# Wu0409/DuPL

Measured on AMD Instinct MI355X. Metric: training img/s at 448^2, VOC dual-student ViT-B/16, phase B step, higher is better.
Workload: dtype f32 storage / accumulation / results; Linear GEMMs (forward, dgrad, wgrad), attention (forward, backward) and the decoder convs as fp32-equivalent f16x3 split products on the f16 MFMA (operands as fp16 hi / lo planes, 3 products per block, fp32 accumulate; error vs fp64 <= the f32 MFMA kernels'); CA

## Files before the change

### dupl_amd/csrc/attn_split.hip

```cpp
#include "split_frag.h"
#include "../../include/dupl_hip.h"

#ifndef ATT_PRIO
#define ATT_PRIO 0
#endif
#ifndef ATT_ABL
#define ATT_ABL 0
#endif

namespace {

constexpr int HD = 64, KT = 64;
constexpr int PLANE = KT * 128;
constexpr int STAGE = 4 * PLANE;

struct AttnSegs {
    int n;
    int row0[DUPL_ATTN_SEGS_MAX], B[DUPL_ATTN_SEGS_MAX], N[DUPL_ATTN_SEGS_MAX], B_f32[DUPL_ATTN_SEGS_MAX], first[DUPL_ATTN_SEGS_MAX + 1];
    float* out[DUPL_ATTN_SEGS_MAX];
    float* lse[DUPL_ATTN_SEGS_MAX];
};

template <class In, class Out>
__device__ __forceinline__ void attn_seg_planes(const size_t r0, const int H, In& qkv_hi, In& qkv_lo, Out& out_hi, Out& out_lo) {
    qkv_hi += r0 * (size_t)(3 * H * HD);
    qkv_lo += r0 * (size_t)(3 * H * HD);
    if (out_hi) { out_hi += r0 * (size_t)(H * HD); out_lo += r0 * (size_t)(H * HD); }
}

__global__ __launch_bounds__(256, 2) void attn_fwd16_kernel(const __half* __restrict__ qkv_hi, const __half* __restrict__ qkv_lo,
                                                            __half* __restrict__ out_hi, __half* __restrict__ out_lo,
                                                            const AttnSegs segs, int H, float scale, int remap, float out_scale) {
    __shared__ __attribute__((aligned(1024))) char smem[2 * STAGE];
    const int tid = threadIdx.x, lane = tid & 63, l31 = lane & 31, hf = lane >> 5;
    const int wave = __builtin_amdgcn_readfirstlane(tid >> 6);
    int sg = 0;
#pragma unroll 1
    while (sg + 1 < segs.n && (int)blockIdx.x >= segs.first[sg + 1]) ++sg;
    sg = __builtin_amdgcn_readfirstlane(sg);
    const int N = segs.N[sg], B_f32 = segs.B_f32[sg];
    float* __restrict__ out = segs.out[sg];
    float* __restrict__ lse = segs.lse[sg];
    int bx, h, b;
    {
        const int gx = (N + 127) / 128;
        const int G = gx * H * segs.B[sg];
        const int L = (int)blockIdx.x - segs.first[sg];
        const int w = remap ? xcd_band(L, G) : L;
        bx = w % gx; h = (w / gx) % H; b = w / (gx * H);
    }
    attn_seg_planes((size_t)segs.row0[sg], H, qkv_hi, qkv_lo, out_hi, out_lo);
    const int q0 = bx * 128 + wave * 32;
    const int D = H * HD, ld = 3 * D;
    const int qrow = q0 + l31;
    const bool wave_active = q0 < N;

    h8 qh[4], ql[4];
    {
        const size_t off = ((size_t)b * N + min(qrow, N - 1)) * ld + h * HD + 8 * hf;
#pragma unroll
        for (int s = 0; s < 4; ++s) {
            qh[s] = load_bfrag(qkv_hi + off, s);
            ql[s] = load_bfrag(qkv_lo + off, s);
        }
    }

    const int prow = lane >> 3;
    const char* kbase[2];
    kbase[0] = reinterpret_cast<const char*>(qkv_hi + (size_t)b * N * ld + D + h * HD);
    kbase[1] = reinterpret_cast<const char*>(qkv_lo + (size_t)b * N * ld + D + h * HD);
    const char* vbase[2];
    vbase[0] = kbase[0] + D * 2;
    vbase[1] = kbase[1] + D * 2;
    int krow[2], kch[2], vrow[2];
    const int vch = km_piece_col_bytes(lane);
#pragma unroll
    for (int j = 0; j < 2; ++j) {
        const int r = 8 * (wave + 4 * j) + prow;
        krow[j] = r;
        kch[j] = rm_piece_col_bytes(lane, r);
        const int q = wave + 4 * j, srow = (lane >> 2) & 7;
        vrow[j] = (q >> 1) * 16 + (srow >> 2) * 8 + (q & 1) * 4 + (srow & 3);
    }
    const size_t tstride = (size_t)KT * ld * 2;
    unsigned koff[2], voff[2];
#pragma unroll
    for (int j = 0; j < 2; ++j) {
        koff[j] = (unsigned)krow[j] * (unsigned)(ld * 2) + kch[j];
        voff[j] = (unsigned)vrow[j] * (unsigned)(ld * 2) + vch;
    }
    auto dma16o = [](const char* ubase, const unsigned off, char* dst) __attribute__((always_inline)) { dma16(ubase + off, dst); };
    auto issue = [&](int t, int buf) __attribute__((always_inline)) {
        char* dst = smem + buf * STAGE + wave * 1024;
        const size_t o = t * tstride;
        if (t * KT + KT <= N) {
#pragma unroll
            for (int i = 0; i < 4; ++i) dma16o(kbase[i >> 1] + o, koff[i & 1], dst + i * 4096);
#pragma unroll
            for (int i = 0; i < 4; ++i) dma16o(vbase[i >> 1] + o, voff[i & 1], dst + (4 + i) * 4096);
        } else {
#pragma unroll
            for (int i = 0; i < 4; ++i)
                dma16o(kbase[i >> 1] + o, (unsigned)(min(t * KT + krow[i & 1], N - 1) - t * KT) * (unsigned)(ld * 2) + kch[i & 1], dst + i * 4096);
#pragma unroll
            for (int i = 0; i < 4; ++i)
                dma16o(vbase[i >> 1] + o, (unsigned)(min(t * KT + vrow[i & 1], N - 1) - t * KT) * (unsigned)(ld * 2) + vch, dst + (4 + i) * 4096);
        }
    };

    const int krow_a = pi_row(l31);
    const int k_off = krow_a * 128, k_sw = (krow_a >> 1) & 7;
    const int vg = lane >> 4, vq = lane & 15;
    const unsigned v_lds = (unsigned)(uintptr_t)((__attribute__((address_space(3))) char*)smem) + 2 * PLANE +
                           ((vg >> 1) * 4 + (vq >> 2)) * 64 + (16 * (vg & 1) + 4 * (vq & 3)) * 2;

    f32x16 oM[2], oX[2];
#pragma unroll
    for (int d = 0; d < 2; ++d)
#pragma unroll
        for (int e = 0; e < 16; ++e) { oM[d][e] = 0.f; oX[d][e] = 0.f; }
    float m_run = -INFINITY, l_run = 0.f;

    const int nkt = (N + KT - 1) / KT;
    long long tph[4] = {0, 0, 0, 0}, tlast = 0;
    constexpr bool ABL16 = ATT_ABL & 16;
    if (ABL16) tlast = clock64();
#define ATT_STAMP(i)                                  \
    if (ABL16) {                                      \
        const long long now_ = clock64();             \
        tph[i] += now_ - tlast;                       \
        tlast = now_;                                 \
    }
    issue(0, 0);
    for (int t = 0; t < nkt; ++t) {
        asm volatile("s_waitcnt vmcnt(0)" ::: "memory");
        __syncthreads();
        if (t + 1 < nkt) issue(t + 1, (t + 1) & 1);
        if (!wave_active) continue;
        const char* st = smem + (t & 1) * STAGE;
        ATT_STAMP(0)

        f32x16 sM[2], sX[2];
        const f32x16 zero16 = {0.f, 0.f, 0.f, 0.f, 0.f, 0.f, 0.f, 0.f, 0.f, 0.f, 0.f, 0.f, 0.f, 0.f, 0.f, 0.f};
        h8 kh[2][2], kl[2][2];
        auto k_read = [&](const int sstep, h8(&fh)[2], h8(&fl)[2]) __attribute__((always_inline)) {
            const int ch = ((2 * sstep + hf) ^ k_sw) * 16;
#pragma unroll
            for (int kt2 = 0; kt2 < 2; ++kt2) {
                fh[kt2] = *reinterpret_cast<const h8*>(st + kt2 * 4096 + k_off + ch);
                fl[kt2] = *reinterpret_cast<const h8*>(st + PLANE + kt2 * 4096 + k_off + ch);
            }
        };
        k_read(0, kh[0], kl[0]);
        __builtin_amdgcn_s_setprio(ATT_PRIO);
#pragma unroll
        for (int sstep = 0; sstep < 4; ++sstep) {
            const int cur = sstep & 1;
            if (sstep + 1 < 4) k_read(sstep + 1, kh[cur ^ 1], kl[cur ^ 1]);
            __builtin_amdgcn_sched_barrier(0);
            sM[0] = MFMA16(kh[cur][0], qh[sstep], sstep == 0 ? zero16 : sM[0]);
            sM[1] = MFMA16(kh[cur][1], qh[sstep], sstep == 0 ? zero16 : sM[1]);
            sX[0] = MFMA16(kh[cur][0], ql[sstep], sstep == 0 ? zero16 : sX[0]);
            sX[1] = MFMA16(kh[cur][1], ql[sstep], sstep == 0 ? zero16 : sX[1]);
            sX[0] = MFMA16(kl[cur][0], qh[sstep], sX[0]);
            sX[1] = MFMA16(kl[cur][1], qh[sstep], sX[1]);
            __builtin_amdgcn_sched_barrier(0);
        }
        __builtin_amdgcn_s_setprio(0);
        if (ATT_ABL & 16) { asm volatile("" ::"v"(sM[0]), "v"(sM[1]), "v"(sX[0]), "v"(sX[1])); }
        ATT_STAMP(1)
        h4 vf[2][8];
        const unsigned v_st = v_lds + (t & 1) * STAGE;
        auto v_read = [&](auto sgc, h4(&f)[8]) __attribute__((always_inline)) {
            constexpr int SG = decltype(sgc)::value;
            static_for<8>([&](auto ic) __attribute__((always_inline)) {
                constexpr int i = decltype(ic)::value, pl = i >> 2, dd = (i >> 1) & 1, jj = i & 1;
                f[i] = km_tr_read<pl * PLANE + ((SG * 2 + jj) * 2 + dd) * 512>(v_st);
            });
        };
        v_read(std::integral_constant<int, 0>{}, vf[0]);
        const float c1 = scale * 1.4426950408889634f, c2 = c1 * LO_INV;
        if (t == nkt - 1) {
            const int kbase_t = t * KT + 8 * hf;
#pragma unroll
            for (int kt2 = 0; kt2 < 2; ++kt2)
#pragma unroll
                for (int e = 0; e < 16; ++e)
                    if (kbase_t + 32 * kt2 + 16 * (e >> 3) + (e & 7) >= N) sM[kt2][e] = -INFINITY;
        }
        float mx = -INFINITY;
#pragma unroll
        for (int kt2 = 0; kt2 < 2; ++kt2)
#pragma unroll
            for (int e = 0; e < 16; ++e) mx = fmaxf(mx, sM[kt2][e]);
        {
            typedef unsigned u2v __attribute__((ext_vector_type(2)));
            const u2v sw = __builtin_amdgcn_permlane32_swap(__float_as_uint(mx), __float_as_uint(mx), false, false);
            mx = fmaxf(__uint_as_float(sw[0]), __uint_as_float(sw[1])) * c1;
        }
        const float m_cand = fmaxf(m_run, mx);
        const bool move = __builtin_amdgcn_ballot_w64(m_cand - m_run > 8.f) != 0;
        const float m_run2 = move ? m_cand : m_run;
        const float m_new = m_run2 == -INFINITY ? 0.f : m_run2;
        const float alpha = __builtin_amdgcn_exp2f(m_run - m_new);
        f32x2 psum2 = {0.f, 0.f};
        h8 ph[4], pl[4];
#pragma unroll
        for (int kt2 = 0; kt2 < 2; ++kt2)
#pragma unroll
            for (int e = 0; e < 16; e += 2) {
                const f32x2 m2 = {sM[kt2][e], sM[kt2][e + 1]}, x2 = {sX[kt2][e], sX[kt2][e + 1]};
                const f32x2 v2 = __builtin_elementwise_fma(x2, f32x2{c2, c2}, __builtin_elementwise_fma(m2, f32x2{c1, c1}, f32x2{-m_new, -m_new}));
                const f32x2 p2 = {__builtin_amdgcn_exp2f(v2[0]), __builtin_amdgcn_exp2f(v2[1])};
                psum2 += p2;
                split_pair(p2, ph[2 * kt2 + (e >> 3)], pl[2 * kt2 + (e >> 3)], e & 7);
            }
        const float psum = psum2[0] + psum2[1];
        l_run = l_run * alpha + psum;
        if (move) {
#pragma unroll
            for (int d = 0; d < 2; ++d)
#pragma unroll
                for (int e = 0; e < 16; ++e) { oM[d][e] *= alpha; oX[d][e] *= alpha; }
        }
        m_run = m_run2;
        if (ATT_ABL & 16) { asm volatile("" ::"v"(ph[0]), "v"(ph[3]), "v"(pl[0]), "v"(pl[3]), "v"(oM[0]), "v"(oX[1])); }
        ATT_STAMP(2)
        __builtin_amdgcn_s_setprio(ATT_PRIO);
        static_for<4>([&](auto sgc) __attribute__((always_inline)) {
            constexpr int sg = decltype(sgc)::value, cur = sg & 1;
            if constexpr (sg + 1 < 4) {
                v_read(std::integral_constant<int, sg + 1>{}, vf[cur ^ 1]);
                asm volatile("s_waitcnt lgkmcnt(8)" ::: "memory");
            } else {
                asm volatile("s_waitcnt lgkmcnt(0)" ::: "memory");
            }
            __builtin_amdgcn_sched_barrier(0);
            const h4(&f)[8] = vf[cur];
            const h8 vh0 = __builtin_shufflevector(f[0], f[1], 0, 1, 2, 3, 4, 5, 6, 7), vh1 = __builtin_shufflevector(f[2], f[3], 0, 1, 2, 3, 4, 5, 6, 7);
            const h8 vl0 = __builtin_shufflevector(f[4], f[5], 0, 1, 2, 3, 4, 5, 6, 7), vl1 = __builtin_shufflevector(f[6], f[7], 0, 1, 2, 3, 4, 5, 6, 7);
            oM[0] = MFMA16(vh0, ph[sg], oM[0]);
            oM[1] = MFMA16(vh1, ph[sg], oM[1]);
            oX[0] = MFMA16(vh0, pl[sg], oX[0]);
            oX[1] = MFMA16(vh1, pl[sg], oX[1]);
            oX[0] = MFMA16(vl0, ph[sg], oX[0]);
            oX[1] = MFMA16(vl1, ph[sg], oX[1]);
            __builtin_amdgcn_sched_barrier(0);
        });
        __builtin_amdgcn_s_setprio(0);
        if (ATT_ABL & 16) { asm volatile("" ::"v"(oM[0]), "v"(oM[1]), "v"(oX[0]), "v"(oX[1])); }
        ATT_STAMP(3)
    }
    if ((ATT_ABL & 16) && lse && tid == 0) {
        long long* q = reinterpret_cast<long long*>(lse + (((size_t)segs.B[sg] * H * N + 1) & ~(size_t)1)) +
                       (size_t)((int)blockIdx.x - segs.first[sg]) * 4;
        q[0] = tph[0]; q[1] = tph[1]; q[2] = tph[2]; q[3] = tph[3];
    }
    if (!wave_active) return;
    const float l_tot = l_run + __shfl_xor(l_run, 32, 64);
    const float inv = 1.f / l_tot;
    if (b >= B_f32) { out = nullptr; lse = nullptr; }
    if (qrow < N) {
        const size_t ro = ((size_t)b * N + qrow) * D + h * HD;
#pragma unroll
        for (int d = 0; d < 2; ++d)
#pragma unroll
            for (int g = 0; g < 4; ++g) {
                float v[4];
#pragma unroll
                for (int j = 0; j < 4; ++j) v[j] = (oM[d][4 * g + j] + oX[d][4 * g + j] * LO_INV) * inv;
                const int col = d * 32 + 8 * g + 4 * hf;
                if (out) *reinterpret_cast<float4*>(out + ro + col) = make_float4(v[0], v[1], v[2], v[3]);
                if (out_hi) {
                    __half hh[4], ll[4];
#pragma unroll
                    for (int j = 0; j < 4; ++j) {
                        if (out_scale > 0.f) split_f32_u(v[j] * out_scale, hh[j], ll[j]);
                        else split_f32(v[j], hh[j], ll[j]);
                    }
                    *reinterpret_cast<uint2*>(out_hi + ro + col) = *reinterpret_cast<const uint2*>(hh);
                    *reinterpret_cast<uint2*>(out_lo + ro + col) = *reinterpret_cast<const uint2*>(ll);
                }
            }
        if (lse && hf == 0) lse[((size_t)b * H + h) * N + qrow] = m_run * 0.6931471805599453f + logf(l_tot);
    }
}

template <int NP>
__global__ __launch_bounds__(256, 2) void attn_fwd16_m16_kernel(const __half* __restrict__ qkv_hi, const __half* __restrict__ qkv_lo,
                                                                __half* __restrict__ out_hi, __half* __restrict__ out_lo,
                                                                const AttnSegs segs, int H, float scale, int remap, float out_scale) {
    static_assert(NP == 1 || NP == 3, "one product or the three of f16x3");
    constexpr bool X = NP == 3;
    constexpr int PL = X ? 2 : 1;
    constexpr int STAGE = 2 * PL * PLANE;
    constexpr bool ABL16 = X && (ATT_ABL & 16);
    __shared__ __attribute__((aligned(1024))) char smem[2 * STAGE];
    const int tid = threadIdx.x, lane = tid & 63, c16 = lane & 15, g4 = lane >> 4;
    const int wave = __builtin_amdgcn_readfirstlane(tid >> 6);
    int sg = 0;
#pragma unroll 1
    while (sg + 1 < segs.n && (int)blockIdx.x >= segs.first[sg + 1]) ++sg;
    sg = __builtin_amdgcn_readfirstlane(sg);
    const int N = segs.N[sg], B_f32 = segs.B_f32[sg];
    float* __restrict__ out = segs.out[sg];
    float* __restrict__ lse = X ? segs.lse[sg] : nullptr;
    int bx, h, b;
    {
        const int gx = (N + 127) / 128;
        const int G = gx * H * segs.B[sg];
        const int L = (int)blockIdx.x - segs.first[sg];
        const int w = remap ? xcd_band(L, G) : L;
        bx = w % gx; h = (w / gx) % H; b = w / (gx * H);
    }
    attn_seg_planes((size_t)segs.row0[sg], H, qkv_hi, qkv_lo, out_hi, out_lo);
    const int q0 = bx * 128 + wave * 32;
    const int D = H * HD, ld = 3 * D;
    const bool wave_active = q0 < N;

    h8 qh[2][2], ql[2][2];
#pragma unroll
    for (int ct = 0; ct < 2; ++ct) {
        const size_t off = ((size_t)b * N + min(q0 + 16 * ct + c16, N - 1)) * ld + h * HD + 8 * g4;
#pragma unroll
        for (int ks = 0; ks < 2; ++ks) {
            qh[ct][ks] = load_bfrag(qkv_hi + off, 2 * ks);
            if constexpr (X) ql[ct][ks] = load_bfrag(qkv_lo + off, 2 * ks);
        }
    }

    const int prow = lane >> 3;
    const char* kbase[2];
    kbase[0] = reinterpret_cast<const char*>(qkv_hi + (size_t)b * N * ld + D + h * HD);
    kbase[1] = reinterpret_cast<const char*>(qkv_lo + (size_t)b * N * ld + D + h * HD);
    const char* vbase[2];
    vbase[0] = kbase[0] + D * 2;
    vbase[1] = kbase[1] + D * 2;
    int krow[2], kch[2], vrow[2];
    const int vch = km16_piece_col_bytes(wave, lane);
#pragma unroll
    for (int j = 0; j < 2; ++j) {
        krow[j] = 8 * (wave + 4 * j) + prow;
        kch[j] = rm16_piece_col_bytes(lane, krow[j]);
        vrow[j] = km16_piece_row(wave + 4 * j, lane);
    }
    const size_t tstride = (size_t)KT * ld * 2;
    unsigned koff[2], voff[2];
#pragma unroll
    for (int j = 0; j < 2; ++j) {
        koff[j] = (unsigned)krow[j] * (unsigned)(ld * 2) + kch[j];
        voff[j] = (unsigned)vrow[j] * (unsigned)(ld * 2) + vch;
    }
    auto dma16o = [](const char* ubase, const unsigned off, char* dst) __attribute__((always_inline)) { dma16(ubase + off, dst); };
    auto issue = [&](int t, int buf) __attribute__((always_inline)) {
        char* dst = smem + buf * STAGE + wave * 1024;
        const size_t o = t * tstride;
        if (t * KT + KT <= N) {
#pragma unroll
            for (int i = 0; i < 2 * PL; ++i) dma16o(kbase[i >> 1] + o, koff[i & 1], dst + i * 4096);
#pragma unroll
            for (int i = 0; i < 2 * PL; ++i) dma16o(vbase[i >> 1] + o, voff[i & 1], dst + (2 * PL + i) * 4096);
        } else {
#pragma unroll
            for (int i = 0; i < 2 * PL; ++i)
                dma16o(kbase[i >> 1] + o, (unsigned)(min(t * KT + krow[i & 1], N - 1) - t * KT) * (unsigned)(ld * 2) + kch[i & 1], dst + i * 4096);
#pragma unroll
            for (int i = 0; i < 2 * PL; ++i)
                dma16o(vbase[i >> 1] + o, (unsigned)(min(t * KT + vrow[i & 1], N - 1) - t * KT) * (unsigned)(ld * 2) + vch, dst + (2 * PL + i) * 4096);
        }
    };

    const int k_off = pi16_row(c16, 0) * 128 + ((g4 ^ rm16_swizzle(pi16_row(c16, 0))) * 16);
    const unsigned v_lds = (unsigned)(uintptr_t)((__attribute__((address_space(3))) char*)smem) + PL * PLANE + km16_read_lane_off(lane);

    f32x4 oM[4][2], oX[4][2];
#pragma unroll
    for (int d = 0; d < 4; ++d)
#pragma unroll
        for (int ct = 0; ct < 2; ++ct) { oM[d][ct] = f32x4{0.f, 0.f, 0.f, 0.f}; oX[d][ct] = f32x4{0.f, 0.f, 0.f, 0.f}; }
    float m_run[2] = {-INFINITY, -INFINITY}, l_run[2] = {0.f, 0.f};

    const int nkt = (N + KT - 1) / KT;
    long long tph[4] = {0, 0, 0, 0}, tlast = 0;
    if (ABL16) tlast = clock64();
    issue(0, 0);
    for (int t = 0; t < nkt; ++t) {
        asm volatile("s_waitcnt vmcnt(0)" ::: "memory");
        __syncthreads();
        if (t + 1 < nkt) issue(t + 1, (t + 1) & 1);
        if (!wave_active) continue;
        const char* st = smem + (t & 1) * STAGE;
        ATT_STAMP(0)

        f32x4 sM[2][2][2], sX[2][2][2];
        const f32x4 zero4 = {0.f, 0.f, 0.f, 0.f};
        h8 kh[2][2], kl[2][2];
        auto k_read = [&](const int step, h8(&fh)[2], h8(&fl)[2]) __attribute__((always_inline)) {
            const int a = (k_off ^ ((step & 1) * 64)) + (step >> 1) * 4096;
#pragma unroll
            for (int j = 0; j < 2; ++j) {
                fh[j] = *reinterpret_cast<const h8*>(st + a + j * 512);
                if constexpr (X) fl[j] = *reinterpret_cast<const h8*>(st + PLANE + a + j * 512);
            }
        };
        k_read(0, kh[0], kl[0]);
        if constexpr (X) __builtin_amdgcn_s_setprio(ATT_PRIO);
#pragma unroll
        for (int step = 0; step < 4; ++step) {
            const int cur = step & 1, G = step >> 1, ks = step & 1;
            if (step + 1 < 4) k_read(step + 1, kh[cur ^ 1], kl[cur ^ 1]);
            __builtin_amdgcn_sched_barrier(0);
#pragma unroll
            for (int j = 0; j < 2; ++j)
#pragma unroll
                for (int ct = 0; ct < 2; ++ct) sM[G][j][ct] = MFMA_16x16x32(kh[cur][j], qh[ct][ks], ks == 0 ? zero4 : sM[G][j][ct]);
            if constexpr (X) {
#pragma unroll
                for (int j = 0; j < 2; ++j)
#pragma unroll
                    for (int ct = 0; ct < 2; ++ct) sX[G][j][ct] = MFMA_16x16x32(kh[cur][j], ql[ct][ks], ks == 0 ? zero4 : sX[G][j][ct]);
#pragma unroll
                for (int j = 0; j < 2; ++j)
#pragma unroll
                    for (int ct = 0; ct < 2; ++ct) sX[G][j][ct] = MFMA_16x16x32(kl[cur][j], qh[ct][ks], sX[G][j][ct]);
            }
            __builtin_amdgcn_sched_barrier(0);
        }
        if constexpr (X) __builtin_amdgcn_s_setprio(0);
        if (ABL16) {
#pragma unroll
            for (int G = 0; G < 2; ++G)
#pragma unroll
                for (int j = 0; j < 2; ++j) asm volatile("" ::"v"(sM[G][j][0]), "v"(sM[G][j][1]), "v"(sX[G][j][0]), "v"(sX[G][j][1]));
        }
        ATT_STAMP(1)
        h4 vf[2][4 * PL];
        const unsigned v_st = v_lds + (t & 1) * STAGE;
        auto v_read = [&](auto hc, h4(&f)[4 * PL]) __attribute__((always_inline)) {
            constexpr int HS = decltype(hc)::value, S = HS >> 1, DH = HS & 1;
            static_for<4 * PL>([&](auto ic) __attribute__((always_inline)) {
                constexpr int i = decltype(ic)::value, pl = i >> 2, dd = (i >> 1) & 1, jj = i & 1;
                f[i] = km_tr_read<pl * PLANE + ((S * 2 + jj) * 4 + 2 * DH + dd) * 512>(v_st);
            });
        };
        v_read(std::integral_constant<int, 0>{}, vf[0]);
        const float c1 = scale * 1.4426950408889634f, c2 = c1 * LO_INV;
        if (t == nkt - 1) {
            const int kbase_t = t * KT + 8 * g4;
#pragma unroll
            for (int G = 0; G < 2; ++G)
#pragma unroll
                for (int j = 0; j < 2; ++j)
#pragma unroll
                    for (int i = 0; i < 4; ++i)
                        if (kbase_t + 32 * G + 4 * j + i >= N) { sM[G][j][0][i] = -INFINITY; sM[G][j][1][i] = -INFINITY; }
        }
        float mxp[2];
        bool want = false;
#pragma unroll
        for (int ct = 0; ct < 2; ++ct) {
            float mx = -INFINITY;
#pragma unroll
            for (int G = 0; G < 2; ++G)
#pragma unroll
                for (int j = 0; j < 2; ++j)
#pragma unroll
                    for (int i = 0; i < 4; ++i) mx = fmaxf(mx, sM[G][j][ct][i]);
            mxp[ct] = mx * c1;
            want = want || (fmaxf(m_run[ct], mxp[ct]) - m_run[ct] > 8.f);
        }
        const bool move = __builtin_amdgcn_ballot_w64(want) != 0;
        if (move) {
#pragma unroll
            for (int ct = 0; ct < 2; ++ct) {
                float mx = mxp[ct];
                mx = fmaxf(mx, __shfl_xor(mx, 16, 64));
                mx = fmaxf(mx, __shfl_xor(mx, 32, 64));
                const float m2 = fmaxf(m_run[ct], mx);
                const float alpha = __builtin_amdgcn_exp2f(m_run[ct] - (m2 == -INFINITY ? 0.f : m2));
                m_run[ct] = m2;
                l_run[ct] *= alpha;
#pragma unroll
                for (int d = 0; d < 4; ++d) {
                    oM[d][ct] *= alpha;
                    if constexpr (X) oX[d][ct] *= alpha;
                }
            }
        }
        h8 ph[2][2], pl[2][2];
#pragma unroll
        for (int ct = 0; ct < 2; ++ct) {
            const float m_new = m_run[ct] == -INFINITY ? 0.f : m_run[ct];
            f32x2 psum2 = {0.f, 0.f};
#pragma unroll
            for (int G = 0; G < 2; ++G)
#pragma unroll
                for (int j = 0; j < 2; ++j)
#pragma unroll
                    for (int i = 0; i < 4; i += 2) {
                        const f32x2 m2 = {sM[G][j][ct][i], sM[G][j][ct][i + 1]};
                        f32x2 v2;
                        if constexpr (X) {
                            const f32x2 x2 = {sX[G][j][ct][i], sX[G][j][ct][i + 1]};
                            v2 = __builtin_elementwise_fma(x2, f32x2{c2, c2}, __builtin_elementwise_fma(m2, f32x2{c1, c1}, f32x2{-m_new, -m_new}));
                        } else v2 = __builtin_elementwise_fma(m2, f32x2{c1, c1}, f32x2{-m_new, -m_new});
                        const f32x2 p2 = {__builtin_amdgcn_exp2f(v2[0]), __builtin_amdgcn_exp2f(v2[1])};
                        psum2 += p2;
                        if constexpr (X) split_pair(p2, ph[G][ct], pl[G][ct], 4 * j + i);
                        else {
                            const h2v hh = __builtin_convertvector(p2, h2v);
                            ph[G][ct][4 * j + i] = hh[0];
                            ph[G][ct][4 * j + i + 1] = hh[1];
                        }
                    }
            l_run[ct] += psum2[0] + psum2[1];
        }
        if (ABL16) {
            asm volatile("" ::"v"(ph[0][0]), "v"(ph[1][1]), "v"(pl[0][0]), "v"(pl[1][1]), "v"(oM[0][0]), "v"(oX[3][1]));
        }
        ATT_STAMP(2)
        if constexpr (X) __builtin_amdgcn_s_setprio(ATT_PRIO);
        static_for<4>([&](auto hc) __attribute__((always_inline)) {
            constexpr int hs = decltype(hc)::value, cur = hs & 1, S = hs >> 1, d0 = 2 * (hs & 1);
            if constexpr (hs + 1 < 4) {
                v_read(std::integral_constant<int, hs + 1>{}, vf[cur ^ 1]);
                if constexpr (X) asm volatile("s_waitcnt lgkmcnt(8)" ::: "memory");
                else asm volatile("s_waitcnt lgkmcnt(4)" ::: "memory");
            } else {
                asm volatile("s_waitcnt lgkmcnt(0)" ::: "memory");
            }
            __builtin_amdgcn_sched_barrier(0);
            const h4(&f)[4 * PL] = vf[cur];
            const h8 vh0 = __builtin_shufflevector(f[0], f[1], 0, 1, 2, 3, 4, 5, 6, 7), vh1 = __builtin_shufflevector(f[2], f[3], 0, 1, 2, 3, 4, 5, 6, 7);
            oM[d0][0] = MFMA_16x16x32(vh0, ph[S][0], oM[d0][0]);
            oM[d0][1] = MFMA_16x16x32(vh0, ph[S][1], oM[d0][1]);
            oM[d0 + 1][0] = MFMA_16x16x32(vh1, ph[S][0], oM[d0 + 1][0]);
            oM[d0 + 1][1] = MFMA_16x16x32(vh1, ph[S][1], oM[d0 + 1][1]);
            if constexpr (X) {
                const h8 vl0 = __builtin_shufflevector(f[4], f[5], 0, 1, 2, 3, 4, 5, 6, 7), vl1 = __builtin_shufflevector(f[6], f[7], 0, 1, 2, 3, 4, 5, 6, 7);
            oX[d0][0] = MFMA_16x16x32(vh0, pl[S][0], oX[d0][0]);
            oX[d0][1] = MFMA_16x16x32(vh0, pl[S][1], oX[d0][1]);
            oX[d0 + 1][0] = MFMA_16x16x32(vh1, pl[S][0], oX[d0 + 1][0]);
            oX[d0 + 1][1] = MFMA_16x16x32(vh1, pl[S][1], oX[d0 + 1][1]);
            oX[d0][0] = MFMA_16x16x32(vl0, ph[S][0], oX[d0][0]);
            oX[d0][1] = MFMA_16x16x32(vl0, ph[S][1], oX[d0][1]);
            oX[d0 + 1][0] = MFMA_16x16x32(vl1, ph[S][0], oX[d0 + 1][0]);
            oX[d0 + 1][1] = MFMA_16x16x32(vl1, ph[S][1], oX[d0 + 1][1]);
            }
            __builtin_amdgcn_sched_barrier(0);
        });
        if constexpr (X) __builtin_amdgcn_s_setprio(0);
        if (ABL16) {
#pragma unroll
            for (int d = 0; d < 4; ++d) asm volatile("" ::"v"(oM[d][0]), "v"(oM[d][1]), "v"(oX[d][0]), "v"(oX[d][1]));
        }
        ATT_STAMP(3)
    }
    if ((ABL16) && lse && tid == 0) {
        long long* q = reinterpret_cast<long long*>(lse + (((size_t)segs.B[sg] * H * N + 1) & ~(size_t)1)) +
                       (size_t)((int)blockIdx.x - segs.first[sg]) * 4;
        q[0] = tph[0]; q[1] = tph[1]; q[2] = tph[2]; q[3] = tph[3];
    }
    if (!wave_active) return;
    if (b >= B_f32) { out = nullptr; lse = nullptr; }
#pragma unroll
    for (int ct = 0; ct < 2; ++ct) {
        float l_tot = l_run[ct];
        l_tot += __shfl_xor(l_tot, 16, 64);
        l_tot += __shfl_xor(l_tot, 32, 64);
        const float inv = 1.f / l_tot;
        const int qrow = q0 + 16 * ct + c16;
        if (qrow < N) {
            const size_t ro = ((size_t)b * N + qrow) * D + h * HD;
#pragma unroll
            for (int d = 0; d < 4; ++d) {
                float v[4];
#pragma unroll
                for (int j = 0; j < 4; ++j) v[j] = (X ? oM[d][ct][j] + oX[d][ct][j] * LO_INV : oM[d][ct][j]) * inv;
                const int col = 16 * d + 4 * g4;
                if (out) *reinterpret_cast<float4*>(out + ro + col) = make_float4(v[0], v[1], v[2], v[3]);
                if (out_hi) {
                    __half hh[4], ll[4];
#pragma unroll
                    for (int j = 0; j < 4; ++j) {
                        if (out_scale > 0.f) split_f32_u(v[j] * out_scale, hh[j], ll[j]);
                        else split_f32(v[j], hh[j], ll[j]);
                    }
                    *reinterpret_cast<uint2*>(out_hi + ro + col) = *reinterpret_cast<const uint2*>(hh);
                    *reinterpret_cast<uint2*>(out_lo + ro + col) = *reinterpret_cast<const uint2*>(ll);
                }
            }
            if (lse && g4 == 0) lse[((size_t)b * H + h) * N + qrow] = m_run[ct] * 0.6931471805599453f + logf(l_tot);
        }
    }
}


}

constexpr int g_attn16_remap = 1;

static int attn_fwd16_launch(const void* qkv_hi, const void* qkv_lo, void* out_hi, void* out_lo, const dupl_attn_seg* sv, int32_t n,
                             int32_t H, int32_t hd, float scale, int32_t out_exp, int32_t mfma, int32_t products, dupl_stream_t s) {
    if (mfma != 0 && mfma != 16 && mfma != 32) return DUPL_ERR_ARG;
    if (products != 1 && products != 3) return DUPL_ERR_ARG;
    const bool single = products == 1;
    if (single && mfma == 32) return DUPL_ERR_ARG;
    if (single && !qkv_lo) qkv_lo = qkv_hi;
    if (out_exp < 0 || out_exp > 15 || !sv || n < 1 || n > DUPL_ATTN_SEGS_MAX) return DUPL_ERR_ARG;
    if (!qkv_hi || !qkv_lo || ((out_hi == nullptr) != (out_lo == nullptr)) || H <= 0 || hd != HD) return DUPL_ERR_ARG;
    auto al16 = [](const void* q) { return (reinterpret_cast<uintptr_t>(q) & 15) == 0; };
    if (!al16(qkv_hi) || !al16(qkv_lo)) return DUPL_ERR_ARG;
    int order[DUPL_ATTN_SEGS_MAX];
    for (int i = 0; i < n; ++i) order[i] = i;
    for (int i = 1; i < n; ++i)
        for (int j = i; j > 0 && sv[order[j]].N > sv[order[j - 1]].N; --j) { const int t = order[j]; order[j] = order[j - 1]; order[j - 1] = t; }
    AttnSegs g;
    g.n = n;
    int total = 0;
    for (int k = 0; k < n; ++k) {
        const dupl_attn_seg& q = sv[order[k]];
        int bf = q.B_f32 == 0 ? q.B : q.B_f32;
        if (q.B <= 0 || q.N <= 0 || q.row0 < 0 || bf < 0 || bf > q.B || (!q.out && !out_hi) || (bf < q.B && q.out && !out_hi)) return DUPL_ERR_ARG;
        if (single && q.lse) return DUPL_ERR_ARG;
        g.row0[k] = (int)q.row0; g.B[k] = q.B; g.N[k] = q.N; g.B_f32[k] = bf; g.out[k] = q.out; g.lse[k] = q.lse;
        g.first[k] = total;
        total += ((q.N + 127) / 128) * H * q.B;
    }
    g.first[n] = total;
    const bool m16 = mfma != 32;
    const float out_scale = out_exp ? ldexpf(1.f, out_exp) : 0.f;
    if (!m16)
        DUPL_LAUNCH(attn_fwd16_kernel, dim3((unsigned)total), dim3(256), 0, (hipStream_t)s, (const __half*)qkv_hi, (const __half*)qkv_lo,
                    (__half*)out_hi, (__half*)out_lo, g, H, scale, g_attn16_remap, out_scale);
    else if (!single)
        DUPL_LAUNCH(attn_fwd16_m16_kernel<3>, dim3((unsigned)total), dim3(256), 0, (hipStream_t)s, (const __half*)qkv_hi, (const __half*)qkv_lo,
                    (__half*)out_hi, (__half*)out_lo, g, H, scale, g_attn16_remap, out_scale);
    else
        DUPL_LAUNCH(attn_fwd16_m16_kernel<1>, dim3((unsigned)total), dim3(256), 0, (hipStream_t)s, (const __half*)qkv_hi, (const __half*)qkv_lo,
                    (__half*)out_hi, (__half*)out_lo, g, H, scale, g_attn16_remap, out_scale);
    return dupl_launch_status();
}

extern "C" int dupl_attention_fwd16_prod(const void* qkv_hi, const void* qkv_lo, float* out, void* out_hi, void* out_lo, float* lse,
                                         int32_t B, int32_t N, int32_t H, int32_t hd, float scale, int32_t B_f32, int32_t out_exp,
                                         int32_t mfma, int32_t products, dupl_stream_t s) {
    if (B_f32 < 0 || B_f32 > B || (B_f32 != 0 && B_f32 < B && !out_hi) || (!out && !out_hi)) return DUPL_ERR_ARG;
    dupl_attn_seg q;
    q.row0 = 0; q.B = B; q.N = N; q.B_f32 = B_f32; q.out = out; q.lse = lse;
    return attn_fwd16_launch(qkv_hi, qkv_lo, out_hi, out_lo, &q, 1, H, hd, scale, out_exp, mfma, products, s);
}

extern "C" int dupl_attention_fwd16_segs_prod(const void* qkv_hi, const void* qkv_lo, void* out_hi, void* out_lo, const dupl_attn_seg* segs,
                                              int32_t n, int32_t H, int32_t hd, float scale, int32_t out_exp, int32_t mfma,
                                              int32_t products, dupl_stream_t s) {
    return attn_fwd16_launch(qkv_hi, qkv_lo, out_hi, out_lo, segs, n, H, hd, scale, out_exp, mfma, products, s);
}

extern "C" int dupl_attention_fwd16_mfma(const void* qkv_hi, const void* qkv_lo, float* out, void* out_hi, void* out_lo, float* lse,
                                         int32_t B, int32_t N, int32_t H, int32_t hd, float scale, int32_t B_f32, int32_t out_exp,
                                         int32_t mfma, dupl_stream_t s) {
    return dupl_attention_fwd16_prod(qkv_hi, qkv_lo, out, out_hi, out_lo, lse, B, N, H, hd, scale, B_f32, out_exp, mfma, 3, s);
}

extern "C" int dupl_attention_fwd16_segs_mfma(const void* qkv_hi, const void* qkv_lo, void* out_hi, void* out_lo, const dupl_attn_seg* segs,
                                              int32_t n, int32_t H, int32_t hd, float scale, int32_t out_exp, int32_t mfma,
                                              dupl_stream_t s) {
    return attn_fwd16_launch(qkv_hi, qkv_lo, out_hi, out_lo, segs, n, H, hd, scale, out_exp, mfma, 3, s);
}

extern "C" int dupl_attention_fwd16(const void* qkv_hi, const void* qkv_lo, float* out, void* out_hi, void* out_lo, float* lse,
                                    int32_t B, int32_t N, int32_t H, int32_t hd, float scale, int32_t B_f32, int32_t out_exp,
                                    dupl_stream_t s) {
    return dupl_attention_fwd16_mfma(qkv_hi, qkv_lo, out, out_hi, out_lo, lse, B, N, H, hd, scale, B_f32, out_exp, 0, s);
}

extern "C" int dupl_attention_fwd16_segs(const void* qkv_hi, const void* qkv_lo, void* out_hi, void* out_lo, const dupl_attn_seg* segs,
                                         int32_t n, int32_t H, int32_t hd, float scale, int32_t out_exp, dupl_stream_t s) {
    return attn_fwd16_launch(qkv_hi, qkv_lo, out_hi, out_lo, segs, n, H, hd, scale, out_exp, 0, 3, s);
}
```

### dupl_amd/csrc/split_frag.h

```cpp
#pragma once
#include "common.h"
#include <type_traits>

namespace {

typedef _Float16 h8 __attribute__((ext_vector_type(8)));
typedef _Float16 h4 __attribute__((ext_vector_type(4)));
typedef _Float16 h2v __attribute__((ext_vector_type(2)));
typedef float f32x2 __attribute__((ext_vector_type(2)));
constexpr float LO_INV = 1.f / DUPL_LO_SCALE;

#define MFMA16(a, b, c) __builtin_amdgcn_mfma_f32_32x32x16_f16((a), (b), (c), 0, 0, 0)
#define MFMA_16x16x32(a, b, c) __builtin_amdgcn_mfma_f32_16x16x32_f16((a), (b), (c), 0, 0, 0)

template <int N, int I = 0, class F>
__device__ __forceinline__ void static_for(F&& f) {
    if constexpr (I < N) {
        f(std::integral_constant<int, I>{});
        static_for<N, I + 1>(f);
    }
}

__device__ __forceinline__ float fast_exp(float x) { return __builtin_amdgcn_exp2f(x * 1.4426950408889634f); }

__device__ __forceinline__ int xcd_band(const int L, const int G) {
    const int q = G >> 3, r = G & 7;
    const int xcd = L & 7, idx = L >> 3;
    return (xcd < r ? xcd * (q + 1) : r * (q + 1) + (xcd - r) * q) + idx;
}
__device__ __forceinline__ void xcd_remap3(int remap, int& bx, int& by, int& bz) {
    bx = blockIdx.x; by = blockIdx.y; bz = blockIdx.z;
    if (!remap) return;
    const int gx = gridDim.x, gy = gridDim.y;
    const int total = gx * gy * gridDim.z;
    const int L = bx + gx * (by + gy * bz);
    const int w = xcd_band(L, total);
    bx = w % gx;
    by = (w / gx) % gy;
    bz = w / (gx * gy);
}

__device__ __forceinline__ void dma16(const char* src, char* dst) {
    __builtin_amdgcn_global_load_lds((const __attribute__((address_space(1))) void*)src,
                                     (__attribute__((address_space(3))) void*)dst, 16, 0, 0);
}

__device__ __forceinline__ int rm_piece_col_bytes(int lane, int row) { return ((lane & 7) ^ ((row >> 1) & 7)) * 16; }

__device__ __forceinline__ int rm16_swizzle(int row) { return ((row >> 1) & 1) | (((row >> 3) & 3) << 1); }
__device__ __forceinline__ int rm16_piece_col_bytes(int lane, int row) { return ((lane & 7) ^ rm16_swizzle(row)) * 16; }

__device__ __forceinline__ int pi_row(int r) {
    const int g = (r >> 2) & 3;
    return (r & ~12) | ((g == 1 ? 2 : (g == 2 ? 1 : g)) << 2);
}

__device__ __forceinline__ int pi16_row(int r, int j) { return 8 * (r >> 2) + 4 * j + (r & 3); }

__device__ __forceinline__ h8 load_bfrag(const __half* p, int s) { return *reinterpret_cast<const h8*>(p + 16 * s); }

__device__ __forceinline__ int km_piece_row(int wave, int lane) {
    const int srow = (lane >> 2) & 7;
    return (wave >> 1) * 16 + (srow >> 2) * 8 + (wave & 1) * 4 + (srow & 3);
}
__device__ __forceinline__ int km_piece_col_bytes(int lane) { return ((lane >> 5) * 32 + (lane & 3) * 8) * 2; }
__device__ __forceinline__ int km_read_lane_off(int lane) {
    const int g = lane >> 4, q = lane & 15;
    return ((g >> 1) * 4 + (q >> 2)) * 64 + (16 * (g & 1) + 4 * (q & 3)) * 2;
}
__device__ __forceinline__ int km16_piece_row(int p, int lane) {
    const int sr = (lane >> 1) & 15;
    return (p >> 2) * 32 + (sr >> 2) * 8 + ((p >> 1) & 1) * 4 + (sr & 3);
}
__device__ __forceinline__ int km16_piece_col_bytes(int p, int lane) { return (16 * (2 * (p & 1) + (lane >> 5)) + 8 * (lane & 1)) * 2; }
__device__ __forceinline__ int km16_read_lane_off(int lane) { return lane * 8; }
template <int OFF>
__device__ __forceinline__ h4 km_tr_read(const unsigned addr) {
    h4 v;
    asm volatile("ds_read_b64_tr_b16 %0, %1 offset:%2" : "=v"(v) : "v"(addr), "n"(OFF) : "memory");
    return v;
}

__device__ __forceinline__ void split_pair(const f32x2 x2, h8& hi, h8& lo, const int i) {
    const h2v hh = __builtin_convertvector(x2, h2v);
    const f32x2 q2 = x2 * f32x2{DUPL_LO_SCALE, DUPL_LO_SCALE};
    hi[i] = hh[0];
    hi[i + 1] = hh[1];
    lo[i] = (_Float16)__builtin_fmaf((float)hh[0], -DUPL_LO_SCALE, q2[0]);
    lo[i + 1] = (_Float16)__builtin_fmaf((float)hh[1], -DUPL_LO_SCALE, q2[1]);
}

}
```

Baseline: 86.85.

## Interleave softmax, max-fold and next-tile DMA into attention forward MFMA phases

```diff
diff --git a/dupl_amd/csrc/attn_split.hip b/dupl_amd/csrc/attn_split.hip
--- a/dupl_amd/csrc/attn_split.hip
+++ b/dupl_amd/csrc/attn_split.hip
@@ -6,6 +6,9 @@
 #endif
 #ifndef ATT_ABL
 #define ATT_ABL 0
+#endif
+#ifndef ATT_SCHED
+#define ATT_SCHED 7
 #endif
 
 namespace {
@@ -286,12 +289,15 @@
     }
 }
 
-template <int NP>
+template <int NP, int SCH>
 __global__ __launch_bounds__(256, 2) void attn_fwd16_m16_kernel(const __half* __restrict__ qkv_hi, const __half* __restrict__ qkv_lo,
                                                                 __half* __restrict__ out_hi, __half* __restrict__ out_lo,
                                                                 const AttnSegs segs, int H, float scale, int remap, float out_scale) {
     static_assert(NP == 1 || NP == 3, "one product or the three of f16x3");
+    static_assert(NP == 3 || SCH == 0, "the single-product form keeps the phase-serial schedule");
     constexpr bool X = NP == 3;
+    constexpr bool SA = SCH & 1, SB = SCH & 2, SC = SCH & 4;
+    constexpr int S_MFMA = 0x008, S_VALU = 0x002, S_TRANS = 0x400;
     constexpr int PL = X ? 2 : 1;
     constexpr int STAGE = 2 * PL * PLANE;
     constexpr bool ABL16 = X && (ATT_ABL & 16);
@@ -369,6 +375,25 @@
                 dma16o(vbase[i >> 1] + o, (unsigned)(min(t * KT + vrow[i & 1], N - 1) - t * KT) * (unsigned)(ld * 2) + vch, dst + (2 * PL + i) * 4096);
         }
     };
+    unsigned ko_n[2] = {0, 0}, vo_n[2] = {0, 0};
+    auto tile_offs = [&](int t) __attribute__((always_inline)) {
+        if (t * KT + KT <= N) {
+#pragma unroll
+            for (int j = 0; j < 2; ++j) { ko_n[j] = koff[j]; vo_n[j] = voff[j]; }
+        } else {
+#pragma unroll
+            for (int j = 0; j < 2; ++j) {
+                ko_n[j] = (unsigned)(min(t * KT + krow[j], N - 1) - t * KT) * (unsigned)(ld * 2) + kch[j];
+                vo_n[j] = (unsigned)(min(t * KT + vrow[j], N - 1) - t * KT) * (unsigned)(ld * 2) + vch;
+            }
+        }
+    };
+    auto dma_piece = [&](const int i, const int t) __attribute__((always_inline)) {
+        char* dst = smem + (t & 1) * STAGE + wave * 1024 + i * 4096;
+        const int p = i & (2 * PL - 1);
+        if (i < 2 * PL) dma16o(kbase[p >> 1] + t * tstride, ko_n[p & 1], dst);
+        else dma16o(vbase[p >> 1] + t * tstride, vo_n[p & 1], dst);
+    };
 
     const int k_off = pi16_row(c16, 0) * 128 + ((g4 ^ rm16_swizzle(pi16_row(c16, 0))) * 16);
     const unsigned v_lds = (unsigned)(uintptr_t)((__attribute__((address_space(3))) char*)smem) + PL * PLANE + km16_read_lane_off(lane);
@@ -387,7 +412,11 @@
     for (int t = 0; t < nkt; ++t) {
         asm volatile("s_waitcnt vmcnt(0)" ::: "memory");
         __syncthreads();
-        if (t + 1 < nkt) issue(t + 1, (t + 1) & 1);
+        const bool more = t + 1 < nkt;
+        if (more) {
+            if (!SC || !wave_active) issue(t + 1, (t + 1) & 1);
+            else tile_offs(t + 1);
+        }
         if (!wave_active) continue;
         const char* st = smem + (t & 1) * STAGE;
         ATT_STAMP(0)
@@ -403,29 +432,58 @@
                 if constexpr (X) fl[j] = *reinterpret_cast<const h8*>(st + PLANE + a + j * 512);
             }
         };
+        auto mask = [&](const int G) __attribute__((always_inline)) {
+            const int kbase_t = t * KT + 8 * g4;
+#pragma unroll
+            for (int j = 0; j < 2; ++j)
+#pragma unroll
+                for (int i = 0; i < 4; ++i)
+                    if (kbase_t + 32 * G + 4 * j + i >= N) { sM[G][j][0][i] = -INFINITY; sM[G][j][1][i] = -INFINITY; }
+        };
+        float mx[2] = {-INFINITY, -INFINITY};
+        auto fold_j = [&](const int G, const int ct, const int j) __attribute__((always_inline)) {
+#pragma unroll
+            for (int i = 0; i < 4; ++i) mx[ct] = fmaxf(mx[ct], sM[G][j][ct][i]);
+        };
+        auto fold = [&](const int G, const int ct) __attribute__((always_inline)) { fold_j(G, ct, 0); fold_j(G, ct, 1); };
+        auto s_ride = [&](auto sc, const int part) __attribute__((always_inline)) {
+            constexpr int step = decltype(sc)::value;
+            if constexpr (SB && step >= 2) {
+                fold_j(0, step - 2, part);
+                static_for<4>([](auto) __attribute__((always_inline)) {
+                    __builtin_amdgcn_sched_group_barrier(S_MFMA, 1, 0);
+                    __builtin_amdgcn_sched_group_barrier(S_VALU, 1, 0);
+                });
+            }
+            if constexpr (SC) {
+                if (more) dma_piece(2 * step + part, t + 1);
+            }
+        };
         k_read(0, kh[0], kl[0]);
         if constexpr (X) __builtin_amdgcn_s_setprio(ATT_PRIO);
-#pragma unroll
-        for (int step = 0; step < 4; ++step) {
-            const int cur = step & 1, G = step >> 1, ks = step & 1;
-            if (step + 1 < 4) k_read(step + 1, kh[cur ^ 1], kl[cur ^ 1]);
+        static_for<4>([&](auto sc) __attribute__((always_inline)) {
+            constexpr int step = decltype(sc)::value, cur = step & 1, G = step >> 1, ks = step & 1;
+            if constexpr (SB && step == 2) { if (t == nkt - 1) mask(0); }
+            if constexpr (step + 1 < 4) k_read(step + 1, kh[cur ^ 1], kl[cur ^ 1]);
             __builtin_amdgcn_sched_barrier(0);
 #pragma unroll
             for (int j = 0; j < 2; ++j)
 #pragma unroll
                 for (int ct = 0; ct < 2; ++ct) sM[G][j][ct] = MFMA_16x16x32(kh[cur][j], qh[ct][ks], ks == 0 ? zero4 : sM[G][j][ct]);
             if constexpr (X) {
+                s_ride(sc, 0);
 #pragma unroll
                 for (int j = 0; j < 2; ++j)
 #pragma unroll
                     for (int ct = 0; ct < 2; ++ct) sX[G][j][ct] = MFMA_16x16x32(kh[cur][j], ql[ct][ks], ks == 0 ? zero4 : sX[G][j][ct]);
+                s_ride(sc, 1);
 #pragma unroll
                 for (int j = 0; j < 2; ++j)
 #pragma unroll
                     for (int ct = 0; ct < 2; ++ct) sX[G][j][ct] = MFMA_16x16x32(kl[cur][j], qh[ct][ks], sX[G][j][ct]);
             }
             __builtin_amdgcn_sched_barrier(0);
-        }
+        });
         if constexpr (X) __builtin_amdgcn_s_setprio(0);
         if (ABL16) {
 #pragma unroll
@@ -446,27 +504,16 @@
         v_read(std::integral_constant<int, 0>{}, vf[0]);
         const float c1 = scale * 1.4426950408889634f, c2 = c1 * LO_INV;
         if (t == nkt - 1) {
-            const int kbase_t = t * KT + 8 * g4;
-#pragma unroll
-            for (int G = 0; G < 2; ++G)
-#pragma unroll
-                for (int j = 0; j < 2; ++j)
-#pragma unroll
-                    for (int i = 0; i < 4; ++i)
-                        if (kbase_t + 32 * G + 4 * j + i >= N) { sM[G][j][0][i] = -INFINITY; sM[G][j][1][i] = -INFINITY; }
+            if constexpr (!SB) mask(0);
+            mask(1);
         }
         float mxp[2];
         bool want = false;
 #pragma unroll
         for (int ct = 0; ct < 2; ++ct) {
-            float mx = -INFINITY;
-#pragma unroll
-            for (int G = 0; G < 2; ++G)
-#pragma unroll
-                for (int j = 0; j < 2; ++j)
-#pragma unroll
-                    for (int i = 0; i < 4; ++i) mx = fmaxf(mx, sM[G][j][ct][i]);
-            mxp[ct] = mx * c1;
+            if constexpr (!SB) fold(0, ct);
+            fold(1, ct);
+            mxp[ct] = mx[ct] * c1;
             want = want || (fmaxf(m_run[ct], mxp[ct]) - m_run[ct] > 8.f);
         }
         const bool move = __builtin_amdgcn_ballot_w64(want) != 0;
@@ -488,24 +535,42 @@
             }
         }
         h8 ph[2][2], pl[2][2];
+        float m_new[2];
+        f32x2 psum2[2];
 #pragma unroll
         for (int ct = 0; ct < 2; ++ct) {
-            const float m_new = m_run[ct] == -INFINITY ? 0.f : m_run[ct];
-            f32x2 psum2 = {0.f, 0.f};
-#pragma unroll
-            for (int G = 0; G < 2; ++G)
-#pragma unroll
-                for (int j = 0; j < 2; ++j)
-#pragma unroll
-                    for (int i = 0; i < 4; i += 2) {
+            m_new[ct] = m_run[ct] == -INFINITY ? 0.f : m_run[ct];
+            psum2[ct] = f32x2{0.f, 0.f};
+        }
+        auto soft = [&](const int G, const int ct) __attribute__((always_inline)) {
+#pragma unroll
+            for (int j = 0; j < 2; ++j)
+#pragma unroll
+                for (int i = 0; i < 4; i += 2) {
+                    if constexpr (SA) {
+                        float p[2];
+#pragma unroll
+                        for (int e = 0; e < 2; ++e) {
+                            float m = sM[G][j][ct][i + e], x = sX[G][j][ct][i + e];
+                            asm("" : "+v"(m));
+                            asm("" : "+v"(x));
+                            float v = __builtin_fmaf(x, c2, __builtin_fmaf(m, c1, -m_new[ct]));
+                            asm("" : "+v"(v));
+                            p[e] = __builtin_amdgcn_exp2f(v);
+                            float acc = psum2[ct][e] + p[e];
+                            asm("" : "+v"(acc));
+                            psum2[ct][e] = acc;
+                        }
+                        split_pair_scalar(p[0], p[1], ph[G][ct], pl[G][ct], 4 * j + i);
+                    } else {
                         const f32x2 m2 = {sM[G][j][ct][i], sM[G][j][ct][i + 1]};
                         f32x2 v2;
                         if constexpr (X) {
                             const f32x2 x2 = {sX[G][j][ct][i], sX[G][j][ct][i + 1]};
-                            v2 = __builtin_elementwise_fma(x2, f32x2{c2, c2}, __builtin_elementwise_fma(m2, f32x2{c1, c1}, f32x2{-m_new, -m_new}));
-                        } else v2 = __builtin_elementwise_fma(m2, f32x2{c1, c1}, f32x2{-m_new, -m_new});
+                            v2 = __builtin_elementwise_fma(x2, f32x2{c2, c2}, __builtin_elementwise_fma(m2, f32x2{c1, c1}, f32x2{-m_new[ct], -m_new[ct]}));
+                        } else v2 = __builtin_elementwise_fma(m2, f32x2{c1, c1}, f32x2{-m_new[ct], -m_new[ct]});
                         const f32x2 p2 = {__builtin_amdgcn_exp2f(v2[0]), __builtin_amdgcn_exp2f(v2[1])};
-                        psum2 += p2;
+                        psum2[ct] += p2;
                         if constexpr (X) split_pair(p2, ph[G][ct], pl[G][ct], 4 * j + i);
                         else {
                             const h2v hh = __builtin_convertvector(p2, h2v);
@@ -513,10 +578,19 @@
                             ph[G][ct][4 * j + i + 1] = hh[1];
                         }
                     }
-            l_run[ct] += psum2[0] + psum2[1];
+                }
+        };
+#pragma unroll
+        for (int ct = 0; ct < 2; ++ct) {
+            soft(0, ct);
+            if constexpr (!SB) soft(1, ct);
+        }
+        if constexpr (!SB) {
+#pragma unroll
+            for (int ct = 0; ct < 2; ++ct) l_run[ct] += psum2[ct][0] + psum2[ct][1];
         }
         if (ABL16) {
-            asm volatile("" ::"v"(ph[0][0]), "v"(ph[1][1]), "v"(pl[0][0]), "v"(pl[1][1]), "v"(oM[0][0]), "v"(oX[3][1]));
+            asm volatile("" ::"v"(ph[0][0]), "v"(ph[SB ? 0 : 1][1]), "v"(pl[0][0]), "v"(pl[SB ? 0 : 1][1]), "v"(oM[0][0]), "v"(oX[3][1]));
         }
         ATT_STAMP(2)
         if constexpr (X) __builtin_amdgcn_s_setprio(ATT_PRIO);
@@ -547,7 +621,26 @@
             oX[d0 + 1][0] = MFMA_16x16x32(vl1, ph[S][0], oX[d0 + 1][0]);
             oX[d0 + 1][1] = MFMA_16x16x32(vl1, ph[S][1], oX[d0 + 1][1]);
             }
+            if constexpr (SB && hs < 2) {
+                soft(1, hs);
+                static_for<4 * NP>([](auto mc) __attribute__((always_inline)) {
+                    __builtin_amdgcn_sched_group_barrier(S_MFMA, 1, 0);
+                    __builtin_amdgcn_sched_group_barrier(S_VALU, 2, 0);
+                    if constexpr (decltype(mc)::value < 8) __builtin_amdgcn_sched_group_barrier(S_TRANS, 1, 0);
+                    __builtin_amdgcn_sched_group_barrier(S_VALU, 3, 0);
+                });
+            }
             __builtin_amdgcn_sched_barrier(0);
+            if constexpr (SB && hs == 1) {
+#pragma unroll
+                for (int ct = 0; ct < 2; ++ct) {
+                    float ps = psum2[ct][0] + psum2[ct][1];
+                    asm("" : "+v"(ps));
+                    float lr = l_run[ct] + ps;
+                    asm("" : "+v"(lr));
+                    l_run[ct] = lr;
+                }
+            }
         });
         if constexpr (X) __builtin_amdgcn_s_setprio(0);
         if (ABL16) {
@@ -602,10 +695,10 @@
 
 static int attn_fwd16_launch(const void* qkv_hi, const void* qkv_lo, void* out_hi, void* out_lo, const dupl_attn_seg* sv, int32_t n,
                              int32_t H, int32_t hd, float scale, int32_t out_exp, int32_t mfma, int32_t products, dupl_stream_t s) {
-    if (mfma != 0 && mfma != 16 && mfma != 32) return DUPL_ERR_ARG;
+    if (mfma != 0 && mfma != 16 && mfma != 18 && mfma != 32) return DUPL_ERR_ARG;
     if (products != 1 && products != 3) return DUPL_ERR_ARG;
     const bool single = products == 1;
-    if (single && mfma == 32) return DUPL_ERR_ARG;
+    if (single && (mfma == 32 || mfma == 18)) return DUPL_ERR_ARG;
     if (single && !qkv_lo) qkv_lo = qkv_hi;
     if (out_exp < 0 || out_exp > 15 || !sv || n < 1 || n > DUPL_ATTN_SEGS_MAX) return DUPL_ERR_ARG;
     if (!qkv_hi || !qkv_lo || ((out_hi == nullptr) != (out_lo == nullptr)) || H <= 0 || hd != HD) return DUPL_ERR_ARG;
@@ -633,11 +726,14 @@
     if (!m16)
         DUPL_LAUNCH(attn_fwd16_kernel, dim3((unsigned)total), dim3(256), 0, (hipStream_t)s, (const __half*)qkv_hi, (const __half*)qkv_lo,
                     (__half*)out_hi, (__half*)out_lo, g, H, scale, g_attn16_remap, out_scale);
+    else if (!single && mfma != 16)
+        DUPL_LAUNCH((attn_fwd16_m16_kernel<3, 0>), dim3((unsigned)total), dim3(256), 0, (hipStream_t)s, (const __half*)qkv_hi, (const __half*)qkv_lo,
+                    (__half*)out_hi, (__half*)out_lo, g, H, scale, g_attn16_remap, out_scale);
     else if (!single)
-        DUPL_LAUNCH(attn_fwd16_m16_kernel<3>, dim3((unsigned)total), dim3(256), 0, (hipStream_t)s, (const __half*)qkv_hi, (const __half*)qkv_lo,
+        DUPL_LAUNCH((attn_fwd16_m16_kernel<3, ATT_SCHED>), dim3((unsigned)total), dim3(256), 0, (hipStream_t)s, (const __half*)qkv_hi, (const __half*)qkv_lo,
                     (__half*)out_hi, (__half*)out_lo, g, H, scale, g_attn16_remap, out_scale);
     else
-        DUPL_LAUNCH(attn_fwd16_m16_kernel<1>, dim3((unsigned)total), dim3(256), 0, (hipStream_t)s, (const __half*)qkv_hi, (const __half*)qkv_lo,
+        DUPL_LAUNCH((attn_fwd16_m16_kernel<1, 0>), dim3((unsigned)total), dim3(256), 0, (hipStream_t)s, (const __half*)qkv_hi, (const __half*)qkv_lo,
                     (__half*)out_hi, (__half*)out_lo, g, H, scale, g_attn16_remap, out_scale);
     return dupl_launch_status();
 }
diff --git a/dupl_amd/csrc/split_frag.h b/dupl_amd/csrc/split_frag.h
--- a/dupl_amd/csrc/split_frag.h
+++ b/dupl_amd/csrc/split_frag.h
@@ -89,5 +89,21 @@
     lo[i] = (_Float16)__builtin_fmaf((float)hh[0], -DUPL_LO_SCALE, q2[0]);
     lo[i + 1] = (_Float16)__builtin_fmaf((float)hh[1], -DUPL_LO_SCALE, q2[1]);
 }
+__device__ __forceinline__ void split_pair_scalar(const float x0, const float x1, h8& hi, h8& lo, const int i) {
+    const h2v hh = __builtin_convertvector(f32x2{x0, x1}, h2v);
+    float q0 = x0 * DUPL_LO_SCALE, q1 = x1 * DUPL_LO_SCALE;
+    float h0 = (float)hh[0], h1 = (float)hh[1];
+    asm("" : "+v"(q0));
+    asm("" : "+v"(q1));
+    asm("" : "+v"(h0));
+    asm("" : "+v"(h1));
+    hi[i] = hh[0];
+    hi[i + 1] = hh[1];
+    float l0 = __builtin_fmaf(h0, -DUPL_LO_SCALE, q0), l1 = __builtin_fmaf(h1, -DUPL_LO_SCALE, q1);
+    asm("" : "+v"(l0));
+    asm("" : "+v"(l1));
+    lo[i] = (_Float16)l0;
+    lo[i + 1] = (_Float16)l1;
+}
 
 }
```

Result: no change. 86.83 (-0.0%).
